# GuanLab/seekmer

Measured on AMD Instinct MI355X. Metric: paired reads/sec mapped+quantified, higher is better.
Workload: dtype u64+f64; 1 GPU; configs[1]: synthetic ~190k-tx index (stand-in for ENSEMBL GRCh38 cDNA), 10000000 2x100bp synthetic pairs per GPU, map+classes+EM to the reference stop rule; transcripts=190402, kmer_slots=134217728, units_per_gpu=10000000, read_len=100, paired=True, classes=851072, class_map_rows=4208693, parallelism=reads sharded x1, RCCL all-reduce f64[T] per EM step, rccl_ranks=0

## Files before the change

### seekmer_amd/csrc/skm_abi.hip

```cpp
#include "../../include/seekmer_hip.h"
#include "skm_kernels.h"
#include "skm_pool.h"
#include "skm_bias.h"
#include "skm_bias_weights.h"

#include <dlfcn.h>
#include <algorithm>
#include <cmath>
#include <cstdarg>
#include <cstdio>
#include <cstdlib>
#include <cstring>
#include <chrono>
#include <condition_variable>
#include <atomic>
#include <deque>
#include <functional>
#include <map>
#include <memory>
#include <unordered_map>
#include <mutex>
#include <thread>
#include <numeric>
#include <string>
// ... 237 lines not shown

struct skm_quant {
    ~skm_quant()
    {
        (void)hipSetDevice(device);
        if (stream) (void)hipStreamSynchronize(stream);
    }
    int device = 0;
    PoolStream stream;
    PoolTimingEvent ev[2];
    PoolEvent chunk_ev[2];
    PoolPinned pinned;
    std::mutex mu;
    int64_t n_tx = 0, n_classes = 0, n_ids = 0, n_rows = 0;
    DBuf<int64_t> cls_offset, row_start, tx_row;
    DBuf<int32_t> ids, tx_cls, row_tx, perm;
    DBuf<double> cls_count, cls_count_saved, inner, row_sum;
    DBuf<double> eff_len, x0, x1, acc, part_max;
    DBuf<unsigned int> part_flags, arrivals;
    DBuf<unsigned long long> ctl, cum;
    DBuf<unsigned int> tile_total;
    DBuf<double> x_start, boot_out;
    struct Batch {
        DBuf<double> cls_count, inner, row_sum, x0, x1, part_max;
        DBuf<unsigned int> part_flags;
        DBuf<unsigned long long> ctl, mgr;
        DBuf<double> counts_all;
        DBuf<double> totals;
        DBuf<int64_t> iters;
    } batch;
    struct Tiles {
        DBuf<int64_t> tile_tx, tile_cls, cls_pair, tx_pair;
        DBuf<int32_t> tx_list, cls_list, tx_label, tx_tile, cls_tile;
        DBuf<uint16_t> cls_tx, tx_cls;
        DBuf<double> snap, step_max;
        DBuf<unsigned int> step_flags;
        struct Residual {
            int64_t n_classes = 0, n_ids = 0, n_rows = 0;
            DBuf<int64_t> cls_offset, row_start, tx_row;
            DBuf<int32_t> ids, cls_src, row_tx, tx_cls;
            DBuf<double> cls_count, inner, row_sum;
            bool built = false;
        } residual;
        bool built = false;
        int64_t n_tiles = 0, n_oversize = 0;
    } tiles;
    double n_total = 0;
    bool n_total_reduced = false;
    void *comm = nullptr;
    int rank = 0, world = 1;
    double t_em_ns = 0, iters_total = 0, launches = 0;
};

struct skm_comm {
    int device = 0;
    void *comm = nullptr;
    int rank = 0, world = 1;
};

extern "C" const char *skm_last_error(void) { return g_error.c_str(); }

extern "C" int skm_device_count(int *count)
{
    if (!count) return fail(SKM_ERR_ARG, "count is NULL");
    int n = 0;
    hipError_t e = hipGetDeviceCount(&n);
// ... 3334 lines not shown
{
    static const bool unfused = getenv("SKM_EM_UNFUSED") != nullptr;
    return !several_ranks && !unfused && em_components_enabled();
}

int quant_alloc(skm_quant *q, int device, int64_t n_tx, int64_t n_classes, int64_t n_ids, bool several_ranks = false)
{
    STALE_CHECK("quant_alloc entry");
    q->device = device;
    q->n_tx = n_tx;
    q->n_classes = n_classes;
    q->n_ids = n_ids;
    HIP_TRY(pool_stream_acquire(q->stream.out()));
    for (auto &e : q->ev) HIP_TRY(pool_event_acquire(e.out(), true));
    for (auto &e : q->chunk_ev) HIP_TRY(pool_event_acquire(e.out(), false));
    HIP_TRY(pool_pinned_acquire((void **)q->pinned.out()));
    const size_t C = (size_t)std::max<int64_t>(n_classes, 1), M = (size_t)std::max<int64_t>(n_ids, 1);
    const size_t T = (size_t)std::max<int64_t>(n_tx, 1);
    const size_t R = (size_t)quant_rows_upper_bound(n_tx, n_ids);
    SKM_TRY(q->cls_offset.ensure(C + 1));
    SKM_TRY(q->cls_count.ensure(C));
    SKM_TRY(q->inner.ensure(C));
    SKM_TRY(q->ids.ensure(M));
    SKM_TRY(q->perm.ensure(C));
    SKM_TRY(q->tx_cls.ensure(M));
    SKM_TRY(q->tx_row.ensure(T + 1));
    SKM_TRY(q->row_start.ensure(R + 1));
    SKM_TRY(q->row_tx.ensure(R));
    SKM_TRY(q->row_sum.ensure(R));
    SKM_TRY(q->eff_len.ensure(T));
    SKM_TRY(q->x0.ensure(T));
    SKM_TRY(q->x1.ensure(T));
    SKM_TRY(q->acc.ensure(T));
    SKM_TRY(q->ctl.ensure(16));
    SKM_TRY(q->part_max.ensure(EM_FINAL_BLOCKS));
    SKM_TRY(q->part_flags.ensure(EM_FINAL_BLOCKS));
    SKM_TRY(q->arrivals.ensure(T));
    HIP_TRY(hipMemsetAsync(q->arrivals.p, 0, T * sizeof(unsigned int), q->stream));
    if (em_tiles_possible(several_ranks)) {
        auto &t = q->tiles;
        SKM_TRY(t.tile_tx.ensure(T + 2)); SKM_TRY(t.tile_cls.ensure(T + 2));
        SKM_TRY(t.cls_pair.ensure(C + 1)); SKM_TRY(t.tx_pair.ensure(T + 1));
        SKM_TRY(t.tx_list.ensure(T)); SKM_TRY(t.cls_list.ensure(C));
        SKM_TRY(t.tx_label.ensure(T)); SKM_TRY(t.tx_tile.ensure(T)); SKM_TRY(t.cls_tile.ensure(C));
        SKM_TRY(t.cls_tx.ensure(M)); SKM_TRY(t.tx_cls.ensure(M));
    }
    STALE_CHECK("quant_alloc exit");
    return SKM_OK;
}

QuantBuild quant_build_view(skm_quant *q)
{
    QuantBuild b{};
    b.n_tx = q->n_tx;
    b.n_classes = q->n_classes;
    b.n_ids = q->n_ids;
    b.cls_offset = q->cls_offset.p;
    b.ids = q->ids.p;
    b.cls_count = q->cls_count.p;
    b.tx_cls = q->tx_cls.p;
    b.tx_row = q->tx_row.p;
    b.row_start = q->row_start.p;
    b.row_tx = q->row_tx.p;
    b.n_rows_cap = (int64_t)q->row_tx.cap;
    if (q->tiles.tile_tx.p) {
        auto &t = q->tiles;
        b.tile_tx = t.tile_tx.p; b.tile_cls = t.tile_cls.p;
        b.tx_list = t.tx_list.p; b.cls_list = t.cls_list.p;
        b.cls_pair = t.cls_pair.p; b.tx_pair = t.tx_pair.p;
        b.tile_cls_tx = t.cls_tx.p; b.tile_tx_cls = t.tx_cls.p;
        b.tx_label = t.tx_label.p; b.tx_tile = t.tx_tile.p; b.cls_tile = t.cls_tile.p;
    }
    return b;
}

int quant_finish_setup(skm_quant *q, const ClassTable *table, int64_t units_seen = -1)
{
    STALE_CHECK("quant_finish_setup");
    QuantBuild b = quant_build_view(q);
    b.first_seen_bound = units_seen > 0 ? units_seen : 0;
    const int64_t rows = quant_setup(table, b, q->perm.p, q->stream);
    if (rows < 0) return fail(SKM_ERR_HIP, "building the class views failed (%lld): %s", (long long)rows, quant_setup_failure());
    q->n_rows = rows;
    if (b.tile_tx) {
        q->tiles.built = true;
        q->tiles.n_tiles = b.tile_info[0];
        q->tiles.n_oversize = b.tile_info[1];
        if (q->tiles.n_tiles > 0) {
            SKM_TRY(q->tiles.step_max.ensure((size_t)(EM_CHUNK_MAX * q->tiles.n_tiles)));
            SKM_TRY(q->tiles.step_flags.ensure((size_t)(EM_CHUNK_MAX * q->tiles.n_tiles)));
            SKM_TRY(q->tiles.snap.ensure((size_t)EM_CHUNK_MAX * (size_t)q->n_tx));
        }
        if (q->tiles.n_oversize > 0 && q->tiles.n_tiles > 0) {
            auto &r = q->tiles.residual;
            int64_t counts[3] = {0, 0, 0};
            if (quant_residual_count(b, counts, q->stream))
                return fail(SKM_ERR_HIP, "sizing the residual EM problem failed: %s", quant_setup_failure());
            r.n_classes = counts[0]; r.n_ids = counts[1]; r.n_rows = counts[2];
            SKM_TRY(r.cls_offset.ensure((size_t)r.n_classes + 1)); SKM_TRY(r.ids.ensure((size_t)std::max<int64_t>(r.n_ids, 1)));
            SKM_TRY(r.cls_src.ensure((size_t)std::max<int64_t>(r.n_classes, 1)));
            SKM_TRY(r.row_start.ensure((size_t)r.n_rows + 1)); SKM_TRY(r.row_tx.ensure((size_t)std::max<int64_t>(r.n_rows, 1)));
            SKM_TRY(r.tx_cls.ensure((size_t)std::max<int64_t>(r.n_ids, 1))); SKM_TRY(r.tx_row.ensure((size_t)q->n_tx + 1));
            SKM_TRY(r.cls_count.ensure((size_t)std::max<int64_t>(r.n_classes, 1)));
            SKM_TRY(r.inner.ensure((size_t)std::max<int64_t>(r.n_classes, 1)));
// ... 99 lines not shown
    return em_tiles_possible(q->comm != nullptr) && q->tiles.built && q->tiles.n_tiles > 0 &&
           (q->tiles.n_oversize == 0 || q->tiles.residual.built);
}

template <class Enqueue, class Stopped>
int em_run_chunks_ahead(skm_quant *q, unsigned long long (&words)[8], Enqueue enqueue, Stopped stopped)
{
    auto enqueue_chunk = [&](int slot) -> int {
        SKM_TRY(enqueue(slot));
        HIP_TRY(hipEventRecord(q->chunk_ev[slot], q->stream));
        return SKM_OK;
    };
    SKM_TRY(enqueue_chunk(0));
    for (int slot = 0;; slot ^= 1) {
        SKM_TRY(enqueue_chunk(slot ^ 1));
        HIP_TRY(hipEventSynchronize(q->chunk_ev[slot]));
        memcpy(words, q->pinned + 8 * slot, sizeof(words));
        if (stopped(words)) return SKM_OK;
    }
}
bool em_ctl_done(const unsigned long long *ctl) { return ctl[CTL_DONE] != 0; }

int em_run_tiles(skm_quant *q, const EmProblem &p, int64_t chunk, int64_t *iters_out)
{
    auto &t = q->tiles;
    EmTiles tl{};
    tl.n_tiles = t.n_tiles;
    tl.tile_tx = t.tile_tx.p; tl.tile_cls = t.tile_cls.p;
    tl.tx_list = t.tx_list.p; tl.cls_list = t.cls_list.p;
    tl.cls_pair = t.cls_pair.p; tl.tx_pair = t.tx_pair.p;
    tl.cls_tx = t.cls_tx.p; tl.tx_cls = t.tx_cls.p;
    tl.step_max = t.step_max.p; tl.step_flags = t.step_flags.p;
    tl.snap = t.snap.p;
    const bool mixed = t.n_oversize > 0;
    EmProblem pr = p;
    if (mixed) {
        auto &r = t.residual;
        pr.n_classes = r.n_classes; pr.n_rows = r.n_rows;
        pr.cls_offset = r.cls_offset.p; pr.ids = r.ids.p; pr.cls_count = r.cls_count.p; pr.inner = r.inner.p;
        pr.row_start = r.row_start.p; pr.row_tx = r.row_tx.p; pr.tx_cls = r.tx_cls.p; pr.tx_row = r.tx_row.p;
        pr.row_sum = r.row_sum.p;
        pr.fused = 1;
        pr.extra_max = t.step_max.p; pr.extra_flags = t.step_flags.p; pr.n_extra = t.n_tiles;
        launch_permute_f64(q->cls_count.p, r.cls_src.p, r.n_classes, r.cls_count.p, false, q->stream);
    }
    int64_t queued = 0;
    auto enqueue_chunk = [&](int slot) -> int {
        launch_em_local_chunk(p, tl, queued == 0 ? q->x0.p : t.snap.p + (chunk - 1) * q->n_tx, (int)chunk, queued * chunk, q->stream);
        if (mixed) {
            pr.extra_first = queued * chunk;
            for (int64_t i = 0, k = queued * chunk; i < chunk; ++i, ++k) {
                launch_em_inner(pr, (int)(k & 1), i > 0, k, q->stream);
                launch_em_rows_finalize(pr, (int)(k & 1), q->stream);
            }
            launch_em_decide(pr, (queued + 1) * chunk, q->stream);
            q->launches += 2 * chunk + 2;
        } else {
            launch_em_local_decide(p, tl, queued * chunk, (int)chunk, q->stream);
            q->launches += 2;
        }
        ++queued;
        HIP_TRY(hipGetLastError());
        HIP_TRY(hipMemcpyAsync(q->pinned + 8 * slot, q->ctl.p, 8 * sizeof(unsigned long long),
                               hipMemcpyDeviceToHost, q->stream));
        return SKM_OK;
    };
    unsigned long long ctl[8] = {0};
    SKM_TRY(em_run_chunks_ahead(q, ctl, enqueue_chunk, em_ctl_done));
    if (ctl[CTL_TILE_FAULT]) {
        HIP_TRY(hipStreamSynchronize(q->stream));
        return fail(SKM_ERR_STATE, "a component tile exceeds the tile capacity: the class views of this handle are damaged");
    }
    const int64_t steps = (int64_t)ctl[CTL_ITERS];
    HIP_TRY(hipEventRecord(q->ev[1], q->stream));
    HIP_TRY(hipEventSynchronize(q->ev[1]));
    float ms = 0;
    HIP_TRY(hipEventElapsedTime(&ms, q->ev[0], q->ev[1]));
    q->t_em_ns += ms * 1e6;
    q->iters_total += (double)steps;
    if (iters_out) *iters_out = steps;
    if (ctl[CTL_UNDEFINED]) return fail(SKM_ERR_UNDEFINED, "no abundance above x_floor: numpy raises on max() of an empty selection");
    return SKM_OK;
}

int em_run(skm_quant *q, double rel_tol, double x_floor, int64_t max_iters, int64_t fixed_iters,
           int64_t *iters_out, int64_t chunk_steps = 16)
{
    double n_total = q->n_total;
    if (q->comm && !q->n_total_reduced) {
        HIP_TRY(hipMemcpyAsync(q->acc.p, &n_total, 8, hipMemcpyHostToDevice, q->stream));
        NCCL_TRY(g_rccl.AllReduce(q->acc.p, q->acc.p, 1, NCCL_FLOAT64, NCCL_SUM, q->comm, q->stream));
        HIP_TRY(hipMemcpyAsync(&n_total, q->acc.p, 8, hipMemcpyDeviceToHost, q->stream));
        HIP_TRY(hipStreamSynchronize(q->stream));
    }
    EmProblem p = em_problem(q, rel_tol, x_floor, max_iters, fixed_iters);
    p.n_total = n_total;
    HIP_TRY(hipMemsetAsync(q->ctl.p, 0, 16 * 8, q->stream));
    int64_t k = 0;
    const int64_t chunk = fixed_iters > 0 ? std::min<int64_t>(fixed_iters, chunk_steps) : chunk_steps;
    HIP_TRY(hipEventRecord(q->ev[0], q->stream));
    if (em_uses_tiles(q) && chunk <= EM_CHUNK_MAX) return em_run_tiles(q, p, chunk, iters_out);
    static const bool unfused_rows = getenv("SKM_EM_UNFUSED") != nullptr;
    auto enqueue_chunk = [&](int slot) -> int {
        for (int64_t i = 0; i < chunk; ++i, ++k) {
            launch_em_inner(p, (int)(k & 1), i > 0, k, q->stream);
            if (q->comm) {
                if (unfused_rows) {
                    launch_em_rows(p, (int)(k & 1), q->stream);
                    launch_em_rows_to_acc(p, q->stream);
                } else {
                    launch_em_rows_acc(p, (int)(k & 1), q->stream);
                }
                NCCL_TRY(g_rccl.AllReduce(q->acc.p, q->acc.p, (size_t)q->n_tx, NCCL_FLOAT64, NCCL_SUM,
                                          q->comm, q->stream));
                launch_em_finalize(p, (int)(k & 1), true, q->stream);
            } else if (p.fused) {
                launch_em_rows_finalize(p, (int)(k & 1), q->stream);
            } else {
                launch_em_rows(p, (int)(k & 1), q->stream);
                launch_em_finalize(p, (int)(k & 1), false, q->stream);
            }
            q->launches += q->comm ? (unfused_rows ? 4 : 3) : (p.fused ? 2 : 3);
        }
        launch_em_decide(p, k, q->stream);
        q->launches += 1;
        HIP_TRY(hipGetLastError());
        HIP_TRY(hipMemcpyAsync(q->pinned + 8 * slot, q->ctl.p, 8 * sizeof(unsigned long long),
                               hipMemcpyDeviceToHost, q->stream));
        return SKM_OK;
    };
// ... 1098 lines not shown
```

### seekmer_amd/csrc/skm_em.hip

```cpp
#include "skm_em_core.h"

namespace skm {

__device__ bool em_evaluate(const EmProblem &p, int n_parts, int64_t steps_done, bool publish);

struct EmWholeTable {
    const EmProblem &p;
    __device__ __forceinline__ int64_t cls_first() const { return 0; }
    __device__ __forceinline__ int64_t cls_end() const { return p.n_classes; }
    __device__ __forceinline__ int64_t row_first() const { return 0; }
    __device__ __forceinline__ int64_t row_end() const { return p.n_rows; }
    __device__ __forceinline__ double n_total() const { return p.n_total; }
    __device__ __forceinline__ bool done() const { return p.ctl[CTL_DONE] != 0; }
    __device__ __forceinline__ bool judge(int eval_parts, int64_t steps_done) const { return em_evaluate(p, eval_parts, steps_done, true); }
    __device__ __forceinline__ int64_t part() const { return blockIdx.x; }
};

__global__ void __launch_bounds__(256)
em_inner_kernel(EmProblem p, int parity, int eval_parts, int64_t steps_done)
{
    em_inner_body(p, EmWholeTable{p}, parity, eval_parts > 0 && blockIdx.x == 0, eval_parts, steps_done, blockIdx.x * (int64_t)blockDim.x + threadIdx.x,
                  (int64_t)gridDim.x * blockDim.x);
}

// ... 66 lines not shown
            m = o > m ? o : m;
            f |= p.extra_flags[first + b];
        }
    }
    if (em_block_reduce<1>(m, f)) {
        const EmVerdict verdict = em_stop_rule(f, m, p.rel_tol, steps_done, p.max_iters, p.fixed_iters);
        if (publish) {
            if (verdict.undefined) p.ctl[CTL_UNDEFINED] = 1;
            p.ctl[CTL_ITERS] = (unsigned long long)steps_done;
            p.ctl[CTL_DONE] = verdict.done ? 1ULL : 0ULL;
        }
        s_done = verdict.done ? 1 : 0;
    }
    __syncthreads();
    return s_done != 0;
}

__global__ void __launch_bounds__(256)
em_decide_kernel(EmProblem p, int n_parts, int64_t steps_done)
{
    if (p.ctl[CTL_DONE]) return;
    em_evaluate(p, n_parts, steps_done, true);
}

#ifndef SKM_EM_TILE_EXPERIMENT
#define SKM_EM_TILE_EXPERIMENT 0
#endif
#ifndef SKM_EM_CLASS_BATCH
#define SKM_EM_CLASS_BATCH 4
#endif
constexpr int EM_CLASS_BATCH = SKM_EM_CLASS_BATCH;
static_assert(EM_CLASS_BATCH == EM_TILE_CLASS_BATCH || EM_CLASS_BATCH == 1, "the set-up orders classes by turns of this width");

__global__ void __launch_bounds__(256)
em_local_chunk_kernel(EmProblem p, EmTiles tl, const double *x_in, int n_steps, int64_t first_step)
{
    static_assert(EM_TILE_TX <= 8 * 32, "a lane group of the row phase takes at most eight transcripts");
    __shared__ double s_x[2][EM_TILE_TX];
    __shared__ double s_eff[EM_TILE_TX];
    __shared__ double s_inner[EM_TILE_CLASSES];
    __shared__ double s_count[EM_TILE_CLASSES];
    __shared__ double s_max[EM_CHUNK_MAX][4];
    __shared__ unsigned int s_flags[EM_CHUNK_MAX][4];
    __shared__ int32_t s_tx[EM_TILE_TX];
    __shared__ uint16_t s_cls_tx[EM_TILE_PAIRS], s_tx_cls[EM_TILE_PAIRS];
    __shared__ uint16_t s_cls_off[EM_TILE_CLASSES + 1], s_tx_off[EM_TILE_TX + 1];
    const int64_t tile = blockIdx.x;
    const int64_t tx0 = tl.tile_tx[tile], cls0 = tl.tile_cls[tile];
    const int n_tx = (int)(tl.tile_tx[tile + 1] - tx0), n_cls = (int)(tl.tile_cls[tile + 1] - cls0);
    const int64_t cp0 = tl.cls_pair[cls0], tp0 = tl.tx_pair[tx0];
    const int n_pairs = (int)(tl.cls_pair[cls0 + n_cls] - cp0);
    if (n_tx > EM_TILE_TX || n_cls > EM_TILE_CLASSES || n_pairs > EM_TILE_PAIRS || n_tx < 0 || n_cls < 0 || n_pairs < 0) {
        if (threadIdx.x == 0) { p.ctl[CTL_TILE_FAULT] = 1; p.ctl[CTL_DONE] = 1; }
        return;
    }
    const int tid = threadIdx.x;
    if (p.ctl[CTL_DONE]) {
        const int64_t steps = (int64_t)p.ctl[CTL_ITERS], at = steps - 1 - (first_step - n_steps);
        if (p.ctl[CTL_TILE_FAULT] || first_step < n_steps || at < 0 || at >= n_steps) return;
        const double *__restrict__ from = tl.snap + at * p.n_tx;
        double *__restrict__ to = p.x[steps & 1];
        for (int i = tid; i < n_tx; i += 256) {
            const int32_t t = tl.tx_list[tx0 + i];
            to[t] = from[t];
        }
        return;
    }
    for (int j = tid; j < n_pairs; j += 256) {
        s_cls_tx[j] = tl.cls_tx[cp0 + j];
        s_tx_cls[j] = tl.tx_cls[tp0 + j];
    }
    for (int k = tid; k <= n_cls; k += 256) {
        s_cls_off[k] = (uint16_t)(tl.cls_pair[cls0 + k] - cp0);
        if (k < n_cls) s_count[k] = p.cls_count[tl.cls_list[cls0 + k]];
        if ((SKM_EM_TILE_EXPERIMENT & 1) && k < n_cls) s_inner[k] = 1.0;
    }
    for (int i = tid; i <= n_tx; i += 256) {
        s_tx_off[i] = (uint16_t)(tl.tx_pair[tx0 + i] - tp0);
        if (i < n_tx) {
            const int32_t t = tl.tx_list[tx0 + i];
// ... 31 lines not shown
                }
                s_inner[k] = s / s_count[k];
            }
        }
        __syncthreads();
        double local_max = 0.0;
        unsigned int flags = 0;
        double my_a = 0.0, my_xt = 0.0;
        int my_i = -1, turn = 0;
        if (!(SKM_EM_TILE_EXPERIMENT & 2)) {
            for (int i = tid >> 3; i < n_tx; i += 32, ++turn) {
                const double xt = x[i];
                const int end = s_tx_off[i + 1];
                int begin = s_tx_off[i];
                double a = 0.0;
                do {
                    const int row_end = min(begin + EM_ROW_CAP, end);
                    a += em_row_sum<false>(s_tx_cls, s_inner, begin, row_end, sub, xt);
                    begin = row_end;
                } while (begin < end);
                if (turn == sub) { my_a = a; my_xt = xt; my_i = i; }
            }
        }
        if (my_i >= 0) {
            const double v = em_new_abundance(my_a, s_eff[my_i], p.n_total);
            x_new[my_i] = v;
            tl.snap[step * p.n_tx + s_tx[my_i]] = v;
            em_note_change(v, my_xt, p.x_floor, local_max, flags);
        }
        em_wave_reduce<1>(local_max, flags);
        if ((tid & 63) == 0) { s_max[step][wave] = local_max; s_flags[step][wave] = flags; }
        __syncthreads();
    }
    if (tid < n_steps) {
        double m;
        unsigned int f;
        em_fold_waves(s_max[tid], s_flags[tid], 1, m, f);
        tl.step_max[tid * tl.n_tiles + tile] = m;
        tl.step_flags[tid * tl.n_tiles + tile] = f;
    }
}

__global__ void __launch_bounds__(64 * EM_CHUNK_MAX)
em_local_decide_kernel(EmProblem p, EmTiles tl, int64_t first_step, int n_steps)
{
    if (p.ctl[CTL_DONE]) return;
    __shared__ double s_max[EM_CHUNK_MAX];
    __shared__ unsigned int s_flags[EM_CHUNK_MAX];
    const int step = threadIdx.x >> 6, lane = threadIdx.x & 63;
    if (step < n_steps) {
        double m = 0.0;
        unsigned int f = 0;
        const double *__restrict__ step_max = tl.step_max + step * tl.n_tiles;
        const unsigned int *__restrict__ step_flags = tl.step_flags + step * tl.n_tiles;
        int64_t b = lane;
        for (; b + 7 * 64 < tl.n_tiles; b += 8 * 64) {
            double o[8];
            unsigned int g[8];
#pragma unroll
            for (int k = 0; k < 8; ++k) { o[k] = step_max[b + 64 * k]; g[k] = step_flags[b + 64 * k]; }
#pragma unroll
            for (int k = 0; k < 8; ++k) { m = o[k] > m ? o[k] : m; f |= g[k]; }
        }
        for (; b < tl.n_tiles; b += 64) {
            const double o = step_max[b];
            m = o > m ? o : m;
            f |= step_flags[b];
        }
        em_wave_reduce<1>(m, f);
        if (lane == 0) { s_max[step] = m; s_flags[step] = f; }
    }
    __syncthreads();
    if (threadIdx.x != 0) return;
    for (int s = 0; s < n_steps; ++s) {
        const int64_t steps_done = first_step + s + 1;
        const EmVerdict verdict = em_stop_rule(s_flags[s], s_max[s], p.rel_tol, steps_done, p.max_iters, p.fixed_iters);
        if (verdict.undefined) p.ctl[CTL_UNDEFINED] = 1;
        p.ctl[CTL_ITERS] = (unsigned long long)steps_done;
        p.ctl[CTL_DONE] = verdict.done ? 1ULL : 0ULL;
        if (verdict.done) break;
    }
}


struct HistogramWeights {
    struct Staged {
        unsigned long long counts[MAX_FRAGMENT_LENGTH];
        unsigned long long part[4];
    };
    const unsigned long long *fld;
    double total;
    __device__ __forceinline__ void stage(int64_t row, Staged &lds)
    {
        fld += row * MAX_FRAGMENT_LENGTH;
        unsigned long long mine = 0;
        for (int i = threadIdx.x; i < MAX_FRAGMENT_LENGTH; i += blockDim.x) {
            lds.counts[i] = fld[i];
            mine += lds.counts[i];
        }
        for (int d = 32; d > 0; d >>= 1) mine += __shfl_xor(mine, d, 64);
        if ((threadIdx.x & 63) == 0) lds.part[threadIdx.x >> 6] = mine;
        __syncthreads();
        total = (double)(long long)(lds.part[0] + lds.part[1] + lds.part[2] + lds.part[3]);
    }
    __device__ __forceinline__ double weight(int i, const Staged &lds) const
    {
        return (double)(long long)lds.counts[i] / total;
    }
};

struct GivenWeights {
    struct Staged {};
    const double *p;
    __device__ __forceinline__ void stage(int64_t row, Staged &) { p += row * MAX_FRAGMENT_LENGTH; }
    __device__ __forceinline__ double weight(int i, const Staged &) const { return p[i]; }
// ... 261 lines not shown
                       judge_previous ? em_final_blocks(p) : 0, steps_done);
}

void launch_em_decide(const EmProblem &p, int64_t steps_done, hipStream_t stream)
{
    hipLaunchKernelGGL(em_decide_kernel, dim3(1), dim3(256), 0, stream, p, em_final_blocks(p), steps_done);
}

void launch_em_rows(const EmProblem &p, int parity, hipStream_t stream)
{
    hipLaunchKernelGGL(em_rows_kernel, dim3(chip_grid(p.n_rows, 32)), dim3(256), 0, stream, p, parity);
}

void launch_em_rows_finalize(const EmProblem &p, int parity, hipStream_t stream)
{
    hipLaunchKernelGGL(em_rows_finalize_kernel<false>, dim3((unsigned)em_final_blocks(p)), dim3(256), 0, stream, p, parity);
}

void launch_em_rows_acc(const EmProblem &p, int parity, hipStream_t stream)
{
    EmProblem fused = p;
    fused.fused = 1;
    hipLaunchKernelGGL(em_rows_finalize_kernel<true>, dim3((unsigned)em_final_blocks(fused)), dim3(256), 0, stream, p, parity);
}

void launch_em_local_chunk(const EmProblem &p, const EmTiles &tiles, const double *x_in, int n_steps, int64_t first_step,
                           hipStream_t stream)
{
    if (tiles.n_tiles <= 0 || n_steps <= 0) return;
    hipLaunchKernelGGL(em_local_chunk_kernel, dim3((unsigned)tiles.n_tiles), dim3(256), 0, stream, p, tiles, x_in,
                       std::min(n_steps, EM_CHUNK_MAX), first_step);
}

void launch_em_local_decide(const EmProblem &p, const EmTiles &tiles, int64_t first_step, int n_steps, hipStream_t stream)
{
    hipLaunchKernelGGL(em_local_decide_kernel, dim3(1), dim3(64 * EM_CHUNK_MAX), 0, stream, p, tiles, first_step,
                       std::min(n_steps, EM_CHUNK_MAX));
}

void launch_em_rows_to_acc(const EmProblem &p, hipStream_t stream)
{
    hipLaunchKernelGGL(em_rows_to_acc_kernel, dim3(chip_grid(p.n_tx, 256)), dim3(256), 0, stream, p);
}

void launch_em_finalize(const EmProblem &p, int parity, bool from_acc, hipStream_t stream)
{
    const int blocks = em_final_blocks(p);
    if (from_acc)
        hipLaunchKernelGGL(em_finalize_kernel<true>, dim3((unsigned)blocks), dim3(256), 0, stream, p, parity);
    else
        hipLaunchKernelGGL(em_finalize_kernel<false>, dim3((unsigned)blocks), dim3(256), 0, stream, p, parity);
}

constexpr int NP_MAX_LEAVES = 160;

__device__ __forceinline__ double np_leaf_sum(const double *a, int n)
{
    if (n < 8) {
        double r = 0.0;
        for (int i = 0; i < n; ++i) r += a[i];
        return r;
    }
    double r[8];
    for (int j = 0; j < 8; ++j) r[j] = a[j];
    int i = 8;
    for (; i < n - (n % 8); i += 8)
        for (int j = 0; j < 8; ++j) r[j] += a[i + j];
    double res = ((r[0] + r[1]) + (r[2] + r[3])) + ((r[4] + r[5]) + (r[6] + r[7]));
    for (; i < n; ++i) res += a[i];
    return res;
}
// ... 289 lines not shown
```

### seekmer_amd/csrc/skm_kernels.h

```cpp
#pragma once
#include "skm_device.h"

namespace skm {

struct MapBatch {
    const uint32_t *records;
    int64_t n_units;
    int32_t words_per_read;
    int32_t record_words;
    int32_t paired;
    int32_t *workspace;
    int32_t *rec_unit;
    uint64_t *rec_key;
    unsigned long long *rec_tuple;
    int32_t keep_spans;
    int32_t *unit_begin, *unit_end;
    Coord *unit_anchor;
    int32_t *unit_entries;
    int64_t ids_capacity;
    int32_t ids_chunk;
    unsigned long long *ids_cursor;
    unsigned long long *fld;
    unsigned long long *stats;
    int32_t vote[8];
// ... 165 lines not shown
                      hipStream_t stream);

#ifndef SKM_EM_TILE_PAIRS
#define SKM_EM_TILE_PAIRS 2048
#endif
#ifndef SKM_EM_TILE_CLASSES
#define SKM_EM_TILE_CLASSES 512
#endif
#ifndef SKM_EM_TILE_TX
#define SKM_EM_TILE_TX 128
#endif
#ifndef SKM_EM_TILE_SEGMENT
#define SKM_EM_TILE_SEGMENT 256
#endif
constexpr int EM_TILE_PAIRS = SKM_EM_TILE_PAIRS, EM_TILE_CLASSES = SKM_EM_TILE_CLASSES, EM_TILE_TX = SKM_EM_TILE_TX;
static_assert(EM_TILE_PAIRS <= 65535 && EM_TILE_CLASSES <= 65535 && EM_TILE_TX <= 65535, "tile-local indices and offsets are 16 bits wide");
constexpr int EM_TILE_SEGMENT = SKM_EM_TILE_SEGMENT;
static_assert(EM_TILE_SEGMENT > 0, "a packing run holds at least one transcript id");
constexpr int EM_CHUNK_MAX = 16;
constexpr int EM_TILE_CLASS_BATCH = 4;
struct EmTiles {
    int64_t n_tiles;
    const int64_t *tile_tx;
    const int64_t *tile_cls;
    const int32_t *tx_list;
    const int32_t *cls_list;
    const int64_t *cls_pair;
    const int64_t *tx_pair;
    const uint16_t *cls_tx;
    const uint16_t *tx_cls;
    double *step_max;
    unsigned int *step_flags;
    double *snap;
};
void launch_em_local_chunk(const EmProblem &p, const EmTiles &tiles, const double *x_in, int n_steps, int64_t first_step,
                           hipStream_t stream);
void launch_em_local_decide(const EmProblem &p, const EmTiles &tiles, int64_t first_step, int n_steps, hipStream_t stream);

constexpr int EM_BATCH = 8;
struct EmBatchProblem {
    int64_t n_tx, n_classes, n_rows;
    const int64_t *cls_offset;
    const int32_t *ids;
    const int64_t *row_start;
    const int32_t *row_tx;
    const int32_t *tx_cls;
    const int64_t *tx_row;
    const double *eff_len;
    const double *cls_count;
    double *inner;
    double *row_sum;
    double *x[2];
    double *place_total;
    double rel_tol, x_floor;
    unsigned long long *ctl;
    double *part_max;
    unsigned int *part_flags;
    int managed;
    unsigned long long *mgr;
    int64_t *iters_out;
    int fused;
    unsigned int *arrivals;
};
enum { BCTL_ALL_DONE = 0, BCTL_LAST_STEP = 1, BCTL_DONE = 8, BCTL_ITERS = 16, BCTL_UNDEFINED = 24 };
enum { MGR_NEXT = 0, MGR_COUNT = 1, MGR_FINISHED = 2, MGR_UNDEFINED = 3, MGR_REP = 8, MGR_SINCE = 16, MGR_TAKE = 24,
       MGR_PUT = 32 };
void launch_em_batch_manage_init(const EmBatchProblem &p, unsigned long long *mgr, unsigned long long *host_pinned64,
                                 int64_t n_reps, const double *counts_all, const double *totals, const double *x_start,
                                 double *out_all, hipStream_t stream);
void launch_em_batch_manage(const EmBatchProblem &p, unsigned long long *mgr, const double *counts_all, const double *totals,
// ... 30 lines not shown
    int64_t max_iters;
    EmSetSlot *slots;
    int n_slots;
    int n_parts;
    double *part_max;
    unsigned int *part_flags;
    unsigned int *arrivals;
};
int em_set_parts(int64_t largest_rows);
void launch_em_set_step(const EmSetProblem &p, int64_t largest_classes, int64_t step, bool judge_previous, hipStream_t stream);
void launch_em_set_decide(const EmSetProblem &p, int64_t steps_done, unsigned long long *running, hipStream_t stream);
void launch_em_set_result(const EmSetSlot *slots, int n_slots, const double *x0, const double *x1, int64_t n_tx, double *out,
                          hipStream_t stream);
void launch_stack_tuples(const int64_t *src, const int64_t *dst, const int32_t *add, int64_t n_classes, const int32_t *arena,
                         int32_t *ids, hipStream_t stream);
void launch_repeat_row(double *x, int64_t n_tx, int64_t n, hipStream_t stream);

struct QuantBuild {
    int64_t n_tx, n_classes, n_ids;
    int64_t *cls_offset;
    int32_t *ids;
    double *cls_count;
    int32_t *tx_cls;
    int64_t *tx_row;
    int64_t *row_start;
    int32_t *row_tx;
    int64_t n_rows_cap;
    int64_t first_seen_bound;
    int64_t *tile_tx, *tile_cls;
    int32_t *tx_list, *cls_list;
    int64_t *cls_pair, *tx_pair;
    uint16_t *tile_cls_tx, *tile_tx_cls;
    int32_t *tx_label, *tx_tile, *cls_tile;
    int64_t tile_info[2];
};
int64_t quant_setup(const ClassTable *table, QuantBuild &q, int32_t *perm, hipStream_t stream);
struct QuantResidual {
    int64_t n_classes, n_ids, n_rows;
    int64_t *cls_offset;
    int32_t *ids;
    int32_t *cls_src;
    int64_t *row_start;
    int32_t *row_tx;
    int32_t *tx_cls;
    int64_t *tx_row;
};
int quant_residual_count(const QuantBuild &q, int64_t counts[3], hipStream_t stream);
int quant_residual_build(const QuantBuild &q, QuantResidual &r, hipStream_t stream);
void launch_permute_f64(const double *x, const int32_t *perm, int64_t n, double *y, bool scatter,
                        hipStream_t stream);
const char *quant_setup_failure();
int64_t quant_rows_upper_bound(int64_t n_tx, int64_t n_ids);

void launch_np_sum(const double *a, int64_t n, double divisor, double *block_sums, double *out,
                   hipStream_t stream);
void launch_np_sum_many(const double *a, int64_t n, int64_t count, int64_t stride, double divisor,
                        double *block_sums, double *out, hipStream_t stream);
void launch_reciprocal(const double *l, int64_t n, double *x, hipStream_t stream);
void launch_divide(double *x, int64_t n, const double *s, bool threshold, double floor, hipStream_t stream);
void launch_divide_many(double *x, int64_t n, int64_t count, int64_t stride, const double *s, bool threshold,
                        double floor, hipStream_t stream);
void launch_effective_lengths(const unsigned long long *fld, const double *lengths, int64_t n_tx,
                              double *out, hipStream_t stream);
void launch_effective_lengths_many(const unsigned long long *fld, int64_t n, const double *lengths, int64_t n_tx,
                                   double *out, hipStream_t stream);
void launch_effective_lengths_weights(const double *p, int64_t n, const double *lengths, int64_t n_tx, double *out,
// ... 100 lines not shown
```

### seekmer_amd/csrc/skm_quant_setup.hip

```cpp
#include "skm_kernels.h"
#include "skm_pool.h"

#include <algorithm>
#include <cstdio>
#include <vector>

namespace skm {

namespace {

struct Scratch {
    hipStream_t stream;
    std::vector<void *> held;
    explicit Scratch(hipStream_t s) : stream(s) {}
    template <class T>
    T *alloc(size_t n)
    {
        void *p = nullptr;
        if (pool_alloc(&p, std::max<size_t>(n, 1) * sizeof(T)) != hipSuccess) return nullptr;
        held.push_back(p);
        return static_cast<T *>(p);
    }
    ~Scratch()
    {
// ... 848 lines not shown
        local[c] = (int32_t)(k - first[min((int64_t)(tile_sorted[k] >> shift), *n_tiles)]);
        len[k] = cls_offset[c + 1] - cls_offset[c];
    }
}

__global__ void __launch_bounds__(256)
tile_fill_cls_kernel(const int32_t *cls_list, int64_t n_classes, const int64_t *cls_offset, const int32_t *ids,
                     const int32_t *tx_local, const int64_t *cls_pair, const int32_t *cls_tile, int32_t residual_tile,
                     uint16_t *out)
{
    for (int64_t k = blockIdx.x * (int64_t)blockDim.x + threadIdx.x; k < n_classes;
         k += (int64_t)gridDim.x * blockDim.x) {
        const int32_t c = cls_list[k];
        if (cls_tile[c] == residual_tile) continue;
        const int64_t src = cls_offset[c], n = cls_offset[c + 1] - src, dst = cls_pair[k];
        for (int64_t j = 0; j < n; ++j) out[dst + j] = (uint16_t)tx_local[ids[src + j]];
    }
}

__global__ void __launch_bounds__(256)
tile_fill_tx_kernel(const int32_t *tx_list, int64_t n_tx, const int64_t *tx_row, const int64_t *row_start,
                    const int32_t *tx_cls, const int32_t *cls_local, const int64_t *tx_pair, const int32_t *tx_tile,
                    uint16_t *out)
{
    const int sub = threadIdx.x & 7;
    for (int64_t i = (blockIdx.x * (int64_t)blockDim.x + threadIdx.x) >> 3; i < n_tx;
         i += ((int64_t)gridDim.x * blockDim.x) >> 3) {
        const int32_t t = tx_list[i];
        if (tx_tile[t] == (int32_t)n_tx) continue;
        const int64_t src = row_start[tx_row[t]], n = row_start[tx_row[t + 1]] - src, dst = tx_pair[i];
        for (int64_t j = sub; j < n; j += 8) out[dst + j] = (uint16_t)cls_local[tx_cls[src + j]];
    }
}

int build_tiles(Scratch &scratch, QuantBuild &q)
{
    hipStream_t stream = scratch.stream;
    const int64_t C = q.n_classes, M = q.n_ids, T = q.n_tx;
    if (M >= (1LL << 31) || C >= (1LL << 31) || T >= (1LL << 31) - 2) return -2;
    const int64_t n_segments = (T + EM_TILE_SEGMENT - 1) / EM_TILE_SEGMENT;
    QB_ALLOC(parent, int32_t, T); QB_ALLOC(comp, int32_t, 3 * T); QB_ALLOC(root_tile, int32_t, T);
    QB_ALLOC(seg_tiles, int64_t, n_segments); QB_ALLOC(seg_base, int64_t, n_segments + 1);
    QB_ALLOC(oversize, unsigned long long, 1);
    QB_ALLOC(iota, int32_t, std::max(T, C)); QB_ALLOC(sorted_tile, int32_t, std::max(T, C));
    QB_ALLOC(tx_local, int32_t, T); QB_ALLOC(cls_local, int32_t, C);
    QB_ALLOC(len, int64_t, std::max(T, C));
    QB_TRY(hipMemsetAsync(comp, 0, 3 * T * sizeof(int32_t), stream));
    QB_TRY(hipMemsetAsync(oversize, 0, sizeof(unsigned long long), stream));
    hipLaunchKernelGGL(iota_kernel, dim3(blocks_for(T)), dim3(256), 0, stream, parent, T);
    hipLaunchKernelGGL(cc_hook_kernel, dim3(blocks_for(C)), dim3(256), 0, stream, q.cls_offset, q.ids, C, parent);
    hipLaunchKernelGGL(cc_label_kernel, dim3(blocks_for(T)), dim3(256), 0, stream, parent, q.tx_row, q.row_start, T,
                       q.tx_label, comp);
    hipLaunchKernelGGL(cc_classes_kernel, dim3(blocks_for(C)), dim3(256), 0, stream, q.cls_offset, q.ids, C,
                       q.tx_label, comp);
    hipLaunchKernelGGL(tile_pack_kernel, dim3(blocks_for(64 * n_segments)), dim3(256), 0, stream, comp, T, n_segments,
                       root_tile, seg_tiles, oversize);
    if (exclusive_scan_with_total(scratch, seg_tiles, seg_base, n_segments)) return -1;
    int end_bit = 1;
    while ((1LL << end_bit) < T + 1 && end_bit < 31) ++end_bit;
    const int degree_bits = end_bit + 5 <= 31 ? 5 : 0;
    QB_ALLOC(tx_key, int32_t, T);
    hipLaunchKernelGGL(tx_tile_kernel, dim3(blocks_for(T)), dim3(256), 0, stream, q.tx_label, root_tile, seg_base, T,
                       q.tx_row, q.row_start, degree_bits, q.tx_tile, tx_key);
    hipLaunchKernelGGL(iota_kernel, dim3(blocks_for(std::max(T, C))), dim3(256), 0, stream, iota, std::max(T, C));
    if (sort_pairs(scratch, tx_key, sorted_tile, iota, q.tx_list, T, end_bit + degree_bits)) return -1;
    hipLaunchKernelGGL(tile_starts_kernel, dim3(blocks_for(T + 1)), dim3(256), 0, stream, sorted_tile, degree_bits, T,
                       seg_base + n_segments, q.tile_tx);
    hipLaunchKernelGGL(tile_local_tx_kernel, dim3(blocks_for(T)), dim3(256), 0, stream, q.tx_list, sorted_tile, degree_bits,
                       q.tile_tx, seg_base + n_segments, T, q.tx_row, q.row_start, tx_local, len);
    if (exclusive_scan_with_total(scratch, len, q.tx_pair, T)) return -1;
    const int length_bits = SKM_EM_CLASS_ORDER ? degree_bits : 0;
    QB_ALLOC(cls_key, int32_t, C);
    hipLaunchKernelGGL(cls_tile_kernel, dim3(blocks_for(C)), dim3(256), 0, stream, q.cls_offset, q.ids, C, q.tx_tile,
                       length_bits, q.cls_tile, cls_key);
    if (sort_pairs(scratch, cls_key, sorted_tile, iota, q.cls_list, C, end_bit + length_bits)) return -1;
    hipLaunchKernelGGL(tile_starts_kernel, dim3(blocks_for(C + 1)), dim3(256), 0, stream, sorted_tile, length_bits, C,
                       seg_base + n_segments, q.tile_cls);
    hipLaunchKernelGGL(tile_local_cls_kernel, dim3(blocks_for(C)), dim3(256), 0, stream, q.cls_list, sorted_tile, length_bits,
                       q.tile_cls, seg_base + n_segments, C, q.cls_offset, cls_local, len);
    if (exclusive_scan_with_total(scratch, len, q.cls_pair, C)) return -1;
    hipLaunchKernelGGL(tile_fill_cls_kernel, dim3(blocks_for(C)), dim3(256), 0, stream, q.cls_list, C, q.cls_offset,
                       q.ids, tx_local, q.cls_pair, q.cls_tile, (int32_t)T, q.tile_cls_tx);
    hipLaunchKernelGGL(tile_fill_tx_kernel, dim3(blocks_for(8 * T)), dim3(256), 0, stream, q.tx_list, T, q.tx_row,
                       q.row_start, q.tx_cls, cls_local, q.tx_pair, q.tx_tile, q.tile_tx_cls);
    QB_TRY(hipMemcpyAsync(&q.tile_info[0], seg_base + n_segments, sizeof(int64_t), hipMemcpyDeviceToHost, stream));
    QB_TRY(hipMemcpyAsync(&q.tile_info[1], oversize, sizeof(int64_t), hipMemcpyDeviceToHost, stream));
    return 0;
}

}

int64_t quant_setup(const ClassTable *table, QuantBuild &q, int32_t *perm, hipStream_t stream)
{
    const bool can_rank = table && q.first_seen_bound > 0 && q.first_seen_bound <= RANK_BITMAP_MAX_UNITS;
    for (int attempt = can_rank ? 0 : 1; attempt < 2; ++attempt) {
        int64_t n_rows = -1;
        {
            Scratch scratch(stream);
            if (attempt == 0) {
                const int rc = build_from_table_ranked(scratch, *table, q, perm);
                if (rc == 1) continue;
                if (rc) return -1;
            } else {
                if (table && build_from_table(scratch, *table, q)) return -1;
                if (localize(scratch, q, perm)) return -1;
            }
            if (transpose(scratch, q)) return -1;
            if (q.tile_tx && build_tiles(scratch, q)) return -1;
            QB_TRY(hipGetLastError());
            QB_TRY(hipMemcpyAsync(&n_rows, q.tx_row + q.n_tx, sizeof(int64_t), hipMemcpyDeviceToHost, stream));
        }
        if (n_rows > q.n_rows_cap) return -3;
        return n_rows;
    }
    return -1;
}

// ... 121 lines not shown
```

Before: 1.000 billion pairs/s.

## Fold EM tile stop decision into last-arriving block and order tiles by fill

Measured after the change: 1.020 billion pairs/s, median of 6. +2.0%, better.

```diff
diff --git a/seekmer_amd/csrc/skm_abi.hip b/seekmer_amd/csrc/skm_abi.hip
--- a/seekmer_amd/csrc/skm_abi.hip
+++ b/seekmer_amd/csrc/skm_abi.hip
@@ -293,6 +293,7 @@
     struct Tiles {
         DBuf<int64_t> tile_tx, tile_cls, cls_pair, tx_pair;
         DBuf<int32_t> tx_list, cls_list, tx_label, tx_tile, cls_tile;
+        DBuf<int32_t> order;
         DBuf<uint16_t> cls_tx, tx_cls;
         DBuf<double> snap, step_max;
         DBuf<unsigned int> step_flags;
@@ -3693,7 +3694,7 @@
     SKM_TRY(q->x0.ensure(T));
     SKM_TRY(q->x1.ensure(T));
     SKM_TRY(q->acc.ensure(T));
-    SKM_TRY(q->ctl.ensure(16));
+    SKM_TRY(q->ctl.ensure(EM_CTL_WORDS + EM_JUDGE_WORDS));
     SKM_TRY(q->part_max.ensure(EM_FINAL_BLOCKS));
     SKM_TRY(q->part_flags.ensure(EM_FINAL_BLOCKS));
     SKM_TRY(q->arrivals.ensure(T));
@@ -3705,6 +3706,7 @@
         SKM_TRY(t.tx_list.ensure(T)); SKM_TRY(t.cls_list.ensure(C));
         SKM_TRY(t.tx_label.ensure(T)); SKM_TRY(t.tx_tile.ensure(T)); SKM_TRY(t.cls_tile.ensure(C));
         SKM_TRY(t.cls_tx.ensure(M)); SKM_TRY(t.tx_cls.ensure(M));
+        SKM_TRY(t.order.ensure(T + 1));
     }
     STALE_CHECK("quant_alloc exit");
     return SKM_OK;
@@ -3731,6 +3733,7 @@
         b.cls_pair = t.cls_pair.p; b.tx_pair = t.tx_pair.p;
         b.tile_cls_tx = t.cls_tx.p; b.tile_tx_cls = t.tx_cls.p;
         b.tx_label = t.tx_label.p; b.tx_tile = t.tx_tile.p; b.cls_tile = t.cls_tile.p;
+        b.tile_order = t.order.p;
     }
     return b;
 }
@@ -3896,7 +3899,14 @@
     tl.cls_tx = t.cls_tx.p; tl.tx_cls = t.tx_cls.p;
     tl.step_max = t.step_max.p; tl.step_flags = t.step_flags.p;
     tl.snap = t.snap.p;
+    tl.order = t.order.p;
+    if (const char *form = getenv("SKM_EM_TILE_ORDER")) {
+        if (!strcmp(form, "identity")) tl.order = nullptr;
+        else if (!strcmp(form, "reverse")) tl.order_reversed = 1;
+        else return fail(SKM_ERR_ARG, "SKM_EM_TILE_ORDER is identity or reverse, not '%s'", form);
+    }
     const bool mixed = t.n_oversize > 0;
+    if (!mixed && !SKM_EM_JUDGE_LAUNCH) tl.judge = q->ctl.p + EM_CTL_WORDS;
     EmProblem pr = p;
     if (mixed) {
         auto &r = t.residual;
@@ -3920,8 +3930,11 @@
             launch_em_decide(pr, (queued + 1) * chunk, q->stream);
             q->launches += 2 * chunk + 2;
         } else {
+#if SKM_EM_JUDGE_LAUNCH
             launch_em_local_decide(p, tl, queued * chunk, (int)chunk, q->stream);
-            q->launches += 2;
+            q->launches += 1;
+#endif
+            q->launches += 1;
         }
         ++queued;
         HIP_TRY(hipGetLastError());
@@ -3959,7 +3972,7 @@
     }
     EmProblem p = em_problem(q, rel_tol, x_floor, max_iters, fixed_iters);
     p.n_total = n_total;
-    HIP_TRY(hipMemsetAsync(q->ctl.p, 0, 16 * 8, q->stream));
+    HIP_TRY(hipMemsetAsync(q->ctl.p, 0, (EM_CTL_WORDS + EM_JUDGE_WORDS) * sizeof(unsigned long long), q->stream));
     int64_t k = 0;
     const int64_t chunk = fixed_iters > 0 ? std::min<int64_t>(fixed_iters, chunk_steps) : chunk_steps;
     HIP_TRY(hipEventRecord(q->ev[0], q->stream));
diff --git a/seekmer_amd/csrc/skm_em.hip b/seekmer_amd/csrc/skm_em.hip
--- a/seekmer_amd/csrc/skm_em.hip
+++ b/seekmer_amd/csrc/skm_em.hip
@@ -122,6 +122,46 @@
 constexpr int EM_CLASS_BATCH = SKM_EM_CLASS_BATCH;
 static_assert(EM_CLASS_BATCH == EM_TILE_CLASS_BATCH || EM_CLASS_BATCH == 1, "the set-up orders classes by turns of this width");
 
+__device__ __forceinline__ unsigned long long em_tile_arrive(unsigned long long *judge, bool has, double m, unsigned int f)
+{
+    if (has) {
+        unsigned long long *word_max = judge + EM_JUDGE_MAX + threadIdx.x, *word_flags = judge + EM_JUDGE_FLAGS + threadIdx.x;
+        const unsigned long long bits = (unsigned long long)__double_as_longlong(m);
+        if (__hip_atomic_load(word_max, __ATOMIC_RELAXED, __HIP_MEMORY_SCOPE_AGENT) < bits)
+            __hip_atomic_fetch_max(word_max, bits, __ATOMIC_RELAXED, __HIP_MEMORY_SCOPE_AGENT);
+        if (f & ~(unsigned int)__hip_atomic_load(word_flags, __ATOMIC_RELAXED, __HIP_MEMORY_SCOPE_AGENT))
+            __hip_atomic_fetch_or(word_flags, (unsigned long long)f, __ATOMIC_RELAXED, __HIP_MEMORY_SCOPE_AGENT);
+    }
+    asm volatile("s_waitcnt vmcnt(0)" ::: "memory");
+    unsigned long long arrived = 0;
+    if (threadIdx.x == 0)
+        arrived = __hip_atomic_fetch_add(judge + EM_JUDGE_ARRIVED, 1ULL, __ATOMIC_RELAXED, __HIP_MEMORY_SCOPE_AGENT) + 1ULL;
+    return __shfl(arrived, 0, 64);
+}
+__device__ __forceinline__ void em_tiles_judge(const EmProblem &p, unsigned long long *judge, bool has, int64_t first_step, int n_steps)
+{
+    double m = 0.0;
+    unsigned int f = 0;
+    if (has) {
+        m = __longlong_as_double((long long)__hip_atomic_exchange(judge + EM_JUDGE_MAX + threadIdx.x, 0ULL, __ATOMIC_RELAXED,
+                                                                 __HIP_MEMORY_SCOPE_AGENT));
+        f = (unsigned int)__hip_atomic_exchange(judge + EM_JUDGE_FLAGS + threadIdx.x, 0ULL, __ATOMIC_RELAXED, __HIP_MEMORY_SCOPE_AGENT);
+    }
+    if (threadIdx.x == 0) __hip_atomic_store(judge + EM_JUDGE_ARRIVED, 0ULL, __ATOMIC_RELAXED, __HIP_MEMORY_SCOPE_AGENT);
+    bool undefined = false, done = false;
+    int64_t steps_done = first_step;
+    for (int s = 0; s < n_steps && !done; ++s) {
+        steps_done = first_step + s + 1;
+        const EmVerdict verdict = em_stop_rule(__shfl(f, s, 64), __shfl(m, s, 64), p.rel_tol, steps_done, p.max_iters, p.fixed_iters);
+        undefined |= verdict.undefined;
+        done = verdict.done;
+    }
+    if (threadIdx.x != 0) return;
+    if (undefined) p.ctl[CTL_UNDEFINED] = 1;
+    p.ctl[CTL_ITERS] = (unsigned long long)steps_done;
+    p.ctl[CTL_DONE] = done ? 1ULL : 0ULL;
+}
+
 __global__ void __launch_bounds__(256)
 em_local_chunk_kernel(EmProblem p, EmTiles tl, const double *x_in, int n_steps, int64_t first_step)
 {
@@ -135,7 +175,7 @@
     __shared__ int32_t s_tx[EM_TILE_TX];
     __shared__ uint16_t s_cls_tx[EM_TILE_PAIRS], s_tx_cls[EM_TILE_PAIRS];
     __shared__ uint16_t s_cls_off[EM_TILE_CLASSES + 1], s_tx_off[EM_TILE_TX + 1];
-    const int64_t tile = blockIdx.x;
+    const int64_t tile = tl.order ? tl.order[tl.order_reversed ? tl.n_tiles - 1 - blockIdx.x : blockIdx.x] : blockIdx.x;
     const int64_t tx0 = tl.tile_tx[tile], cls0 = tl.tile_cls[tile];
     const int n_tx = (int)(tl.tile_tx[tile + 1] - tx0), n_cls = (int)(tl.tile_cls[tile + 1] - cls0);
     const int64_t cp0 = tl.cls_pair[cls0], tp0 = tl.tx_pair[tx0];
@@ -233,15 +273,22 @@
         if ((tid & 63) == 0) { s_max[step][wave] = local_max; s_flags[step][wave] = flags; }
         __syncthreads();
     }
-    if (tid < n_steps) {
-        double m;
-        unsigned int f;
-        em_fold_waves(s_max[tid], s_flags[tid], 1, m, f);
-        tl.step_max[tid * tl.n_tiles + tile] = m;
-        tl.step_flags[tid * tl.n_tiles + tile] = f;
-    }
-}
-
+    if (tid >= 64) return;
+    double m = 0.0;
+    unsigned int f = 0;
+    if (tid < n_steps) em_fold_waves(s_max[tid], s_flags[tid], 1, m, f);
+    if (tl.judge == nullptr) {
+        if (tid < n_steps) {
+            tl.step_max[tid * tl.n_tiles + tile] = m;
+            tl.step_flags[tid * tl.n_tiles + tile] = f;
+        }
+        return;
+    }
+    if (em_tile_arrive(tl.judge, tid < n_steps, m, f) != (unsigned long long)tl.n_tiles) return;
+    em_tiles_judge(p, tl.judge, tid < n_steps, first_step, n_steps);
+}
+
+#if SKM_EM_JUDGE_LAUNCH
 __global__ void __launch_bounds__(64 * EM_CHUNK_MAX)
 em_local_decide_kernel(EmProblem p, EmTiles tl, int64_t first_step, int n_steps)
 {
@@ -282,6 +329,7 @@
         if (verdict.done) break;
     }
 }
+#endif
 
 
 struct HistogramWeights {
@@ -609,11 +657,13 @@
                        std::min(n_steps, EM_CHUNK_MAX), first_step);
 }
 
+#if SKM_EM_JUDGE_LAUNCH
 void launch_em_local_decide(const EmProblem &p, const EmTiles &tiles, int64_t first_step, int n_steps, hipStream_t stream)
 {
     hipLaunchKernelGGL(em_local_decide_kernel, dim3(1), dim3(64 * EM_CHUNK_MAX), 0, stream, p, tiles, first_step,
                        std::min(n_steps, EM_CHUNK_MAX));
 }
+#endif
 
 void launch_em_rows_to_acc(const EmProblem &p, hipStream_t stream)
 {
diff --git a/seekmer_amd/csrc/skm_kernels.h b/seekmer_amd/csrc/skm_kernels.h
--- a/seekmer_amd/csrc/skm_kernels.h
+++ b/seekmer_amd/csrc/skm_kernels.h
@@ -221,10 +221,21 @@
     double *step_max;
     unsigned int *step_flags;
     double *snap;
-};
+    const int32_t *order;
+    int32_t order_reversed;
+    unsigned long long *judge;
+};
+enum { EM_JUDGE_MAX = 0, EM_JUDGE_FLAGS = 16, EM_JUDGE_ARRIVED = 32, EM_JUDGE_WORDS = 48 };
+static_assert(EM_CHUNK_MAX <= 16, "a step's word of each kind");
+constexpr int EM_CTL_WORDS = 16;
+#ifndef SKM_EM_JUDGE_LAUNCH
+#define SKM_EM_JUDGE_LAUNCH 0
+#endif
 void launch_em_local_chunk(const EmProblem &p, const EmTiles &tiles, const double *x_in, int n_steps, int64_t first_step,
                            hipStream_t stream);
+#if SKM_EM_JUDGE_LAUNCH
 void launch_em_local_decide(const EmProblem &p, const EmTiles &tiles, int64_t first_step, int n_steps, hipStream_t stream);
+#endif
 
 constexpr int EM_BATCH = 8;
 struct EmBatchProblem {
@@ -321,6 +332,7 @@
     int64_t *cls_pair, *tx_pair;
     uint16_t *tile_cls_tx, *tile_tx_cls;
     int32_t *tx_label, *tx_tile, *cls_tile;
+    int32_t *tile_order;
     int64_t tile_info[2];
 };
 int64_t quant_setup(const ClassTable *table, QuantBuild &q, int32_t *perm, hipStream_t stream);
diff --git a/seekmer_amd/csrc/skm_quant_setup.hip b/seekmer_amd/csrc/skm_quant_setup.hip
--- a/seekmer_amd/csrc/skm_quant_setup.hip
+++ b/seekmer_amd/csrc/skm_quant_setup.hip
@@ -904,6 +904,39 @@
         for (int64_t j = sub; j < n; j += 8) out[dst + j] = (uint16_t)cls_local[tx_cls[src + j]];
     }
 }
+
+constexpr int TILE_ORDER_BINS = 256;
+__global__ void __launch_bounds__(1024)
+tile_order_kernel(const int64_t *__restrict__ tile_cls, const int64_t *__restrict__ cls_pair, const int64_t *n_tiles,
+                  int32_t *__restrict__ order)
+{
+    __shared__ unsigned int at[TILE_ORDER_BINS];
+    const int64_t tiles = *n_tiles;
+    auto bin_of = [&](int64_t i) {
+        const int64_t pairs = cls_pair[tile_cls[i + 1]] - cls_pair[tile_cls[i]];
+        const int64_t fill = min(max(pairs, (int64_t)0), (int64_t)EM_TILE_PAIRS) * (TILE_ORDER_BINS - 1) / EM_TILE_PAIRS;
+        return TILE_ORDER_BINS - 1 - (int)fill;
+    };
+    for (int d = threadIdx.x; d < TILE_ORDER_BINS; d += 1024) at[d] = 0;
+    __syncthreads();
+    for (int64_t i = threadIdx.x; i < tiles; i += 1024) atomicAdd(&at[bin_of(i)], 1u);
+    __syncthreads();
+    if (threadIdx.x < 64) {
+        constexpr int PER = TILE_ORDER_BINS / 64;
+        unsigned int n[PER], sum = 0;
+        for (int k = 0; k < PER; ++k) { n[k] = at[threadIdx.x * PER + k]; sum += n[k]; }
+        unsigned int incl = sum;
+        for (int d = 1; d < 64; d <<= 1) {
+            const unsigned int o = __shfl_up(incl, d, 64);
+            if ((int)threadIdx.x >= d) incl += o;
+        }
+        unsigned int first = incl - sum;
+        for (int k = 0; k < PER; ++k) { at[threadIdx.x * PER + k] = first; first += n[k]; }
+    }
+    __syncthreads();
+    for (int64_t i = threadIdx.x; i < tiles; i += 1024) order[atomicAdd(&at[bin_of(i)], 1u)] = (int32_t)i;
+}
+static_assert(TILE_ORDER_BINS % 64 == 0, "the scan gives every lane of a wave the same number of bins");
 
 int build_tiles(Scratch &scratch, QuantBuild &q)
 {
@@ -955,6 +988,8 @@
                        q.ids, tx_local, q.cls_pair, q.cls_tile, (int32_t)T, q.tile_cls_tx);
     hipLaunchKernelGGL(tile_fill_tx_kernel, dim3(blocks_for(8 * T)), dim3(256), 0, stream, q.tx_list, T, q.tx_row,
                        q.row_start, q.tx_cls, cls_local, q.tx_pair, q.tx_tile, q.tile_tx_cls);
+    hipLaunchKernelGGL(tile_order_kernel, dim3(1), dim3(1024), 0, stream, q.tile_cls, q.cls_pair, seg_base + n_segments,
+                       q.tile_order);
     QB_TRY(hipMemcpyAsync(&q.tile_info[0], seg_base + n_segments, sizeof(int64_t), hipMemcpyDeviceToHost, stream));
     QB_TRY(hipMemcpyAsync(&q.tile_info[1], oversize, sizeof(int64_t), hipMemcpyDeviceToHost, stream));
     return 0;
```
